# radiocosmology/draco

Hardware: AMD Instinct MI355X
Metric: m-modes/sec through MModeTransform+DirtyMapMaker (128-feed, 256-freq) (higher is better)
Workload: dtype f64 accumulate; B stored complex128; FFT complex64 (as the reference); 1 GPU; cfg3: 128-feed (379 stacked baselines), 256 freq per GPU (256 in the job), 1024 RA, lmax=mmax=512: MModeTransform.process + DirtyMapMaker.process through the task classes (131328 (m,f) solves + alm2map to nside=256 IQUV maps per GPU and day); parallelism=freq-sharded x1, weak scaling (no collective in the timed region)

## Files before the change

draco_amd/csrc/dmm_ctx.hip:

```cpp
#include <stdio.h>
#include <string.h>

#include "dmm_internal.h"

static thread_local char g_err[512] = "";

int dmm_set_error(int code, const char* fmt, ...) {
  va_list ap;
  va_start(ap, fmt);
  vsnprintf(g_err, sizeof(g_err), fmt, ap);
  va_end(ap);
  return code;
}

static const char* const kProfNames[DMM_PROF_NSLOT] = {"gram", "chol", "tridiag", "ql", "backproj", "band", "chase", "solve", "null"};

static void prof_collect(dmm_ctx* c) {
  for (dmm_prof_span& sp : c->prof_open) {
    float ms = 0.f;
    if (hipEventSynchronize(sp.b) == hipSuccess && hipEventElapsedTime(&ms, sp.a, sp.b) == hipSuccess) {
      c->prof_us[sp.slot] += 1e3 * (double)ms;
      ++c->prof_n[sp.slot];
    }
    (void)hipEventDestroy(sp.a);
    (void)hipEventDestroy(sp.b);
  }
  c->prof_open.clear();
}

int dmm_get_scratch(dmm_ctx* ctx, size_t bytes, void** out) {
  if (ctx->scratch_bytes < bytes) {
    if (ctx->scratch) {
      DMM_HIP(hipStreamSynchronize(ctx->stream));
      (void)hipFree(ctx->scratch);
      ctx->scratch = nullptr;
      ctx->scratch_bytes = 0;
    }
    DMM_HIP(hipMalloc(&ctx->scratch, bytes));
    ctx->scratch_bytes = bytes;
  }
  *out = ctx->scratch;
  return DMM_OK;
}

hipError_t dmm_ticket(dmm_ctx* ctx, unsigned long long** out) {
  constexpr int kTickets = 256;
  if (!ctx->ticket) {
    hipError_t e = hipMalloc((void**)&ctx->ticket, kTickets * sizeof(unsigned long long));
    if (e != hipSuccess) return e;
  }
  *out = ctx->ticket + (ctx->ticket_seq++ % kTickets);
  return hipSuccess;
}

extern "C" {

int dmm_version(void) { return DMM_VERSION; }
const char* dmm_last_error(void) { return g_err; }

int dmm_ctx_create(int device, dmm_ctx** out) {
  DMM_REQUIRE(out != nullptr, "dmm_ctx_create: ctx is NULL");
  *out = nullptr;
  int ndev = 0;
  DMM_HIP(hipGetDeviceCount(&ndev));
  DMM_REQUIRE(device >= 0 && device < ndev, "dmm_ctx_create: device %d out of range (%d devices)", device, ndev);
  DMM_HIP(hipSetDevice(device));
  dmm_ctx* c = new (std::nothrow) dmm_ctx();
  if (!c) return dmm_set_error(DMM_E_NOMEM, "dmm_ctx_create: out of host memory");
  c->device = device;
  hipDeviceProp_t prop;
  DMM_HIP(hipGetDeviceProperties(&prop, device));
  c->num_cu = prop.multiProcessorCount > 0 ? prop.multiProcessorCount : 256;
  DMM_HIP(hipEventCreate(&c->ev0));
  DMM_HIP(hipEventCreate(&c->ev1));
  *out = c;
  return DMM_OK;
}

static void free_tables(std::map<int, dmm_fft_tables>& m) {
  for (auto& kv : m) {
    if (kv.second.tw) (void)hipFree(kv.second.tw);
    if (kv.second.chirp) (void)hipFree(kv.second.chirp);
    if (kv.second.bfilt) (void)hipFree(kv.second.bfilt);
  }
  m.clear();
}

int dmm_ctx_destroy(dmm_ctx* c) {
  if (!c) return DMM_OK;
  (void)hipSetDevice(c->device);
  free_tables(c->fft);
  free_tables(c->ifft);
  for (auto& kv : c->sht)
    if (kv.second) (void)hipFree(kv.second);
  prof_collect(c);
  if (c->scratch) (void)hipFree(c->scratch);
  if (c->ticket) (void)hipFree(c->ticket);
  if (c->ev0) (void)hipEventDestroy(c->ev0);
  if (c->ev1) (void)hipEventDestroy(c->ev1);
  for (hipEvent_t e : c->aux_ev)
    if (e) (void)hipEventDestroy(e);
  if (c->aux_stream) (void)hipStreamDestroy(c->aux_stream);
  if (c->aux_stream_b) (void)hipStreamDestroy(c->aux_stream_b);
  if (c->aux_pinned) (void)hipHostFree(c->aux_pinned);
  delete c;
  return DMM_OK;
}

int dmm_ctx_set_stream(dmm_ctx* c, void* s) {
  DMM_REQUIRE(c != nullptr, "dmm_ctx_set_stream: ctx is NULL");
  c->stream = (hipStream_t)s;
  return DMM_OK;
}

int dmm_ctx_set_option(dmm_ctx* c, const char* name, int64_t value) {
  DMM_REQUIRE(c != nullptr && name != nullptr, "dmm_ctx_set_option: NULL argument");
  if (!strcmp(name, "dirty_variant")) c->opt_dirty_variant = (int)value;
  else if (!strcmp(name, "grid_mult")) c->opt_grid_mult = (int)value;
  else if (!strcmp(name, "dirty_static")) c->opt_dirty_static = (int)value;
  else if (!strcmp(name, "dirty_nofill")) c->opt_dirty_nofill = (int)value;
  else if (!strcmp(name, "project_grid_mult")) c->opt_project_grid_mult = (int)value;
  else if (!strcmp(name, "project_variant")) c->opt_project_variant = (int)value;
  else if (!strcmp(name, "ml_inner_sweeps")) c->opt_ml_inner_sweeps = (int)value;
  else if (!strcmp(name, "ml_outer_sweeps")) c->opt_ml_outer_sweeps = (int)value;
  else if (!strcmp(name, "sht_variant")) c->opt_sht_variant = (int)value;
  else if (!strcmp(name, "sht_synth_form")) c->opt_sht_synth_form = (int)value;
  else if (!strcmp(name, "ml_shortcut")) c->opt_ml_shortcut = (int)value;
  else if (!strcmp(name, "ml_null")) c->opt_ml_null = (int)value;
  else if (!strcmp(name, "ml_rank_stop")) c->opt_ml_rank_stop = (int)value;
  else if (!strcmp(name, "ml_chase_split")) c->opt_ml_chase_split = (int)value;
  else if (!strcmp(name, "dirty_prio")) c->opt_dirty_prio = (int)value;
  else if (!strcmp(name, "ml_eigen")) c->opt_ml_eigen = (int)value;
  else if (!strcmp(name, "ringmap_variant")) c->opt_ringmap_variant = (int)value;
  else if (!strcmp(name, "ml_reduce")) c->opt_ml_reduce = (int)value;
  else if (!strcmp(name, "gram_stage")) c->opt_gram_stage = (int)value;
  else if (!strcmp(name, "wiener_overlap")) c->opt_wiener_overlap = (int)value;
  else if (!strcmp(name, "ml_workspace_mib")) c->opt_ml_ws_mib = value > 0 ? value : 0;
  else if (!strcmp(name, "regrid_workspace_mib")) c->opt_regrid_ws_mib = value > 0 ? value : 0;
  else if (!strcmp(name, "wiener_workspace_mib")) c->opt_wiener_ws_mib = value > 0 ? value : 0;
  else if (!strcmp(name, "profile")) {
    prof_collect(c);
    for (int k = 0; k < DMM_PROF_NSLOT; ++k) c->prof_us[k] = 0.0, c->prof_n[k] = 0;
    c->opt_profile = value != 0;
  }
  else return dmm_set_error(DMM_E_ARG, "dmm_ctx_set_option: unknown option '%s'", name);
  return DMM_OK;
}

int dmm_ctx_get_counter(dmm_ctx* c, const char* name, int64_t* value) {
  DMM_REQUIRE(c != nullptr && name != nullptr && value != nullptr, "dmm_ctx_get_counter: NULL argument");
  if (!strcmp(name, "ml_tiles_direct")) *value = c->ml_tiles_direct;
  else if (!strcmp(name, "ml_tiles_eigen")) *value = c->ml_tiles_eigen;
  else if (!strcmp(name, "ml_tiles_null")) *value = c->ml_tiles_null;
  else if (!strcmp(name, "ml_tiles_stopped")) *value = c->ml_tiles_stopped;
  else if (!strcmp(name, "ml_gram_cached")) *value = c->ml_gram_cached;
  else if (!strcmp(name, "ml_tiles_basis")) *value = c->ml_tiles_basis;
  else if (!strcmp(name, "ml_stop_cols")) *value = c->ml_stop_cols;
  else if (!strcmp(name, "ml_gram_flops")) *value = c->ml_gram_flops;
  else if (!strcmp(name, "ml_band_bytes")) *value = c->ml_band_bytes;
  else if (!strcmp(name, "ml_tiles_ql_failed")) *value = c->ml_tiles_ql_failed;
  else if (!strcmp(name, "ml_early_chunks")) *value = c->ml_early_chunks;
  else if (!strcmp(name, "ml_two_stage_max_order")) *value = dmm_ml_two_stage_max_order();
  else if (!strcmp(name, "build_ab")) {
#ifdef DMM_AB
    *value = 1;
#else
    *value = 0;
#endif
  }
  else if (!strcmp(name, "opt_sht_synth_form")) *value = c->opt_sht_synth_form;
  else if (!strncmp(name, "prof_", 5)) {
    const size_t len = strlen(name);
    const bool want_n = len > 7 && !strcmp(name + len - 2, "_n");
    const bool want_us = len > 8 && !strcmp(name + len - 3, "_us");
    int slot = -1;
    for (int k = 0; k < DMM_PROF_NSLOT; ++k) {
      const size_t nl = strlen(kProfNames[k]);
      if (!strncmp(name + 5, kProfNames[k], nl) && name[5 + nl] == '_' && 5 + nl + (want_n ? 2 : 3) == len) slot = k;
    }
    if (slot < 0 || !(want_n || want_us)) return dmm_set_error(DMM_E_ARG, "dmm_ctx_get_counter: unknown counter '%s'", name);
    prof_collect(c);
    *value = want_n ? c->prof_n[slot] : (int64_t)(c->prof_us[slot] + 0.5);
  }
  else return dmm_set_error(DMM_E_ARG, "dmm_ctx_get_counter: unknown counter '%s'", name);
  return DMM_OK;
}

int dmm_ctx_set_ml_basis(dmm_ctx* c, void* U, double* sigma, int32_t* rank, int64_t nslots, int rmax, int build) {
  DMM_REQUIRE(c != nullptr, "dmm_ctx_set_ml_basis: ctx is NULL");
  DMM_REQUIRE(U == nullptr || (sigma != nullptr && rank != nullptr && nslots > 0 && rmax >= 64 && rmax % 64 == 0),
              "dmm_ctx_set_ml_basis: a basis needs sigma, rank, a slot count and rmax a multiple of 64");
  c->ml_bs_U = (double2*)U;
  c->ml_bs_sigma = U ? sigma : nullptr;
  c->ml_bs_rank = U ? rank : nullptr;
  c->ml_bs_slots = U ? nslots : 0;
  c->ml_bs_rmax = U ? rmax : 0;
  c->ml_bs_build = U ? (build == 1) : 0;
  c->ml_bs_rank_h.clear();
  if (U && build == 1) {
    DMM_HIP(hipMemsetAsync(rank, 0xFF, (size_t)nslots * sizeof(int32_t), c->stream));
    c->ml_bs_rank_cache_src = nullptr;
  }
  if (U && build != 1) {
    if (build == 0 && c->ml_bs_rank_cache_src == rank && (int64_t)c->ml_bs_rank_cache.size() == nslots) {
      c->ml_bs_rank_h = c->ml_bs_rank_cache;
    } else {
      c->ml_bs_rank_h.resize((size_t)nslots);
      DMM_HIP(hipMemcpyAsync(c->ml_bs_rank_h.data(), rank, (size_t)nslots * sizeof(int32_t), hipMemcpyDeviceToHost, c->stream));
      DMM_HIP(hipStreamSynchronize(c->stream));
      c->ml_bs_rank_cache = c->ml_bs_rank_h;
      c->ml_bs_rank_cache_src = rank;
    }
  }
  return DMM_OK;
}

int dmm_ctx_set_ml_gram_cache(dmm_ctx* c, void* cache, int32_t* valid, int64_t nslots, int reset) {
  DMM_REQUIRE(c != nullptr, "dmm_ctx_set_ml_gram_cache: ctx is NULL");
  DMM_REQUIRE(cache == nullptr || (valid != nullptr && nslots > 0), "dmm_ctx_set_ml_gram_cache: a cache needs its valid flags and a slot count");
  c->ml_gcache = (double2*)cache;
  c->ml_gvalid = cache ? valid : nullptr;
  c->ml_gslots = cache ? nslots : 0;
  if (cache && reset) DMM_HIP(hipMemsetAsync(valid, 0, (size_t)nslots * sizeof(int32_t), c->stream));
  if (cache && (reset || cache != c->ml_gcache_last || (int64_t)c->ml_gvalid_h.size() != nslots)) c->ml_gvalid_h.assign((size_t)nslots, 0);
  if (cache) c->ml_gcache_last = cache;
  return DMM_OK;
}

int dmm_ctx_set_ml_diag(dmm_ctx* c, double* diag) {
  DMM_REQUIRE(c != nullptr, "dmm_ctx_set_ml_diag: ctx is NULL");
  c->ml_diag = diag;
  return DMM_OK;
}

int dmm_ctx_sync(dmm_ctx* c) {
  DMM_REQUIRE(c != nullptr, "dmm_ctx_sync: ctx is NULL");
  DMM_HIP(hipStreamSynchronize(c->stream));
  if (c->aux_stream) DMM_HIP(hipStreamSynchronize(c->aux_stream));
  if (c->aux_stream_b) DMM_HIP(hipStreamSynchronize(c->aux_stream_b));
  return DMM_OK;
}

int dmm_timer_start(dmm_ctx* c) {
  DMM_REQUIRE(c != nullptr, "dmm_timer_start: ctx is NULL");
  DMM_HIP(hipEventRecord(c->ev0, c->stream));
  return DMM_OK;
}

int dmm_timer_stop(dmm_ctx* c, float* ms) {
  DMM_REQUIRE(c != nullptr && ms != nullptr, "dmm_timer_stop: NULL argument");
  DMM_HIP(hipEventRecord(c->ev1, c->stream));
  DMM_HIP(hipEventSynchronize(c->ev1));
  DMM_HIP(hipEventElapsedTime(ms, c->ev0, c->ev1));
  return DMM_OK;
}

}
```

draco_amd/csrc/dmm_internal.h:

```cpp
#pragma once
#include <hip/hip_runtime.h>
#include <stdint.h>
#include <stdarg.h>
#include <map>
#include <vector>

#include "draco_amd.h"

struct dmm_fft_tables {
  int n = 0;
  int M = 0;
  float2* tw = nullptr;
  float2* chirp = nullptr;
  float2* bfilt = nullptr;
};

enum dmm_prof_slot { DMM_PROF_GRAM = 0, DMM_PROF_CHOL, DMM_PROF_TRIDIAG, DMM_PROF_QL, DMM_PROF_BACKPROJ, DMM_PROF_BAND, DMM_PROF_CHASE, DMM_PROF_SOLVE, DMM_PROF_NULL, DMM_PROF_NSLOT };
struct dmm_prof_span {
  hipEvent_t a, b;
  int slot;
};

struct dmm_ctx {
  int device = 0;
  hipStream_t stream = nullptr;
  hipEvent_t ev0 = nullptr, ev1 = nullptr;
  hipStream_t aux_stream = nullptr;
  hipStream_t aux_stream_b = nullptr;
  hipEvent_t aux_ev[4] = {nullptr, nullptr, nullptr, nullptr};
  int* aux_pinned = nullptr;
  size_t aux_pinned_n = 0;
  int num_cu = 256;
  std::map<int, dmm_fft_tables> fft;
  std::map<int, dmm_fft_tables> ifft;
  std::map<int64_t, void*> sht;
  int opt_dirty_variant = 0;
  int opt_grid_mult = 0;
  int opt_dirty_prio = 0;
  int opt_dirty_static = 0;
  int opt_dirty_nofill = 0;
  int opt_project_grid_mult = 0;
  int opt_project_variant = 0;
  int opt_ml_inner_sweeps = 0, opt_ml_outer_sweeps = 0;
  int opt_sht_variant = 0;
  int opt_sht_synth_form = 0;
  int opt_ml_eigen = 0;
  int64_t opt_regrid_ws_mib = 0;
  int64_t opt_ml_ws_mib = 0, opt_wiener_ws_mib = 0;
  int opt_ml_shortcut = 0;
  int ml_probe_every = 8;
  double ml_pass_rate = 1.0;
  int opt_ml_null = 0;
  int64_t ml_gram_flops = 0, ml_band_bytes = 0;
  int64_t ml_tiles_null = 0;
  int opt_ml_chase_split = 0;
  int opt_ml_rank_stop = 0;
  int64_t ml_order_hist[17] = {};
  int64_t ml_tiles_stopped = 0, ml_stop_cols = 0;
  int64_t ml_tiles_direct = 0, ml_tiles_eigen = 0;
  int64_t ml_tiles_ql_failed = 0;
  int opt_ringmap_variant = 0;
  int opt_wiener_overlap = 1;
  int opt_gram_stage = 0;
  int opt_ml_reduce = 0;
  double2* ml_bs_U = nullptr;
  double* ml_bs_sigma = nullptr;
  int32_t* ml_bs_rank = nullptr;
  int64_t ml_bs_slots = 0;
  int ml_bs_rmax = 0, ml_bs_build = 0;
  std::vector<int32_t> ml_bs_rank_h;
  std::vector<int32_t> ml_bs_rank_cache;
  const int32_t* ml_bs_rank_cache_src = nullptr;
  int64_t ml_tiles_basis = 0;
  double2* ml_gcache = nullptr;
  int32_t* ml_gvalid = nullptr;
  int64_t ml_gslots = 0;
  const void* ml_gcache_last = nullptr;
  std::vector<char> ml_gvalid_h;
  int64_t ml_gram_cached = 0;
  double* ml_diag = nullptr;
  int opt_profile = 0;
  std::vector<dmm_prof_span> prof_open;
  double prof_us[DMM_PROF_NSLOT] = {};
  int64_t prof_n[DMM_PROF_NSLOT] = {};
  int64_t ml_early_chunks = 0;
  unsigned long long* ticket = nullptr;
  unsigned ticket_seq = 0;
  void* scratch = nullptr;
  size_t scratch_bytes = 0;
};

int dmm_get_scratch(dmm_ctx* ctx, size_t bytes, void** out);
hipError_t dmm_ticket(dmm_ctx* ctx, unsigned long long** out);

struct dmm_plan {
  dmm_ctx* ctx = nullptr;
  int64_t ntile = 0;
  int npairs = 0, npol = 0, lmax = 0, nfreq = 0, n_m = 0, b_dtype = 0, b_layout = 0;
  std::vector<dmm_tile> tiles_h;
  dmm_tile* tiles_d = nullptr;
  int32_t* work_start_d = nullptr;
  int32_t* work_rows_d = nullptr;
  int64_t nwork = 0, nwork_rows = 0;
  int cols_per_block = 0;
  int pair_ok = 0;
  int64_t b_bytes = 0;
  std::vector<int16_t> ml_ne;
};

struct dmm_aux_scope {
  dmm_ctx* c;
  explicit dmm_aux_scope(dmm_ctx* ctx) : c(ctx) {}
  dmm_aux_scope(const dmm_aux_scope&) = delete;
  dmm_aux_scope& operator=(const dmm_aux_scope&) = delete;
  ~dmm_aux_scope() {
    if (c && c->aux_stream) (void)hipStreamSynchronize(c->aux_stream);
    if (c && c->aux_stream_b) (void)hipStreamSynchronize(c->aux_stream_b);
  }
};

struct dmm_prof_scope {
  dmm_ctx* c;
  hipStream_t st;
  dmm_prof_span sp;
  bool on;
  dmm_prof_scope(dmm_ctx* ctx, int slot, hipStream_t stream) : c(ctx), st(stream), on(false) {
    if (!c->opt_profile) return;
    sp.slot = slot;
    if (hipEventCreate(&sp.a) != hipSuccess) return;
    if (hipEventCreate(&sp.b) != hipSuccess) {
      (void)hipEventDestroy(sp.a);
      return;
    }
    (void)hipEventRecord(sp.a, st);
    on = true;
  }
  dmm_prof_scope(const dmm_prof_scope&) = delete;
  dmm_prof_scope& operator=(const dmm_prof_scope&) = delete;
  ~dmm_prof_scope() {
    if (!on) return;
    (void)hipEventRecord(sp.b, st);
    c->prof_open.push_back(sp);
  }
};

int dmm_set_error(int code, const char* fmt, ...);
#define DMM_HIP(call)                                                                  \
  do {                                                                                 \
    hipError_t e_ = (call);                                                            \
    if (e_ != hipSuccess)                                                              \
      return dmm_set_error((int)e_, "%s failed: %s (%s:%d)", #call, hipGetErrorString(e_), \
                           __FILE__, __LINE__);                                        \
  } while (0)
#define DMM_REQUIRE(cond, ...)                                \
  do {                                                        \
    if (!(cond)) return dmm_set_error(DMM_E_ARG, __VA_ARGS__); \
  } while (0)

int dmm_fft_tables_f64(dmm_ctx* ctx, int n, dmm_fft_tables** out);
void dmm_dirty_tile_list(const dmm_plan* pl, const int64_t* ids, int n, std::vector<dmm_tile>& tiles, std::vector<int32_t>& work);
int dmm_dirty_launch_list(dmm_plan* pl, const void* B, const void* mvis, const double* mweight, const dmm_tile* tiles_d,
                          const int32_t* work_d, int nmat, int64_t nwork, void* alm);
int dmm_dirty_w_launch_list(dmm_plan* pl, const void* B, const double2* wbuf, const double* Sl, const dmm_tile* tiles_d,
                            const int32_t* work_d, int nmat, int64_t nwork, void* alm);
int dmm_ml_two_stage_max_order();

static inline bool dmm_is_pow2(int n) { return n > 0 && (n & (n - 1)) == 0; }
static inline int ilog2(int n) {
  int l = 0;
  while ((1 << l) < n) ++l;
  return l;
}
```

draco_amd/csrc/sht.hip:

```cpp
#include "sht_common.h"
#include "sht_legendre.h"
#include "sht_rings.h"

namespace {

int get_geom(dmm_ctx* ctx, int nside, int lmax, int mmax, ShtGeom* out) {
  const int64_t key = ((int64_t)nside << 40) | ((int64_t)lmax << 20) | (int64_t)mmax;
  auto it = ctx->sht.find(key);
  const int nring = 4 * nside - 1;
  const size_t nd = (size_t)3 * nring + (mmax + 1);
  const size_t bytes = nd * sizeof(double) + (size_t)nring * sizeof(int64_t) + (size_t)nring * sizeof(int);
  const size_t coef_ofs = (bytes + 63) / 64 * 64;
  const size_t coef_rows = (size_t)coef_row0(mmax + 1, lmax);
  int blue_rmax = 0;
  std::vector<int64_t> bf_off(1, 0);
  int64_t bf_total = 0;
  for (int ir = 1; ir < nside && blue_len(ir) <= kMaxBlue; ++ir) {
    bf_off.push_back(bf_total);
    bf_total += blue_len(ir);
    blue_rmax = ir;
  }
  const size_t bfo_ofs = coef_ofs + coef_rows * sizeof(Coef);
  const size_t bf_ofs = (bfo_ofs + bf_off.size() * sizeof(int64_t) + 63) / 64 * 64;
  const size_t phase_ofs = (bf_ofs + (size_t)bf_total * sizeof(double2) + 63) / 64 * 64;
// ... 90 lines not shown
  g.blue_rmax = blue_rmax;
  g.phase = reinterpret_cast<double2*>(gb + phase_ofs);
  g.tw = reinterpret_cast<double2*>(gb + tw_ofs);
  g.tw_len = tw_len;
  g.chirp = reinterpret_cast<double2*>(gb + chirp_ofs);
  *out = g;
  return DMM_OK;
}

int check_args(const char* who, dmm_ctx* ctx, const void* a, const void* b, int nfreq, int npol, int lmax, int mmax,
               int nside) {
  DMM_REQUIRE(ctx && a && b, "%s: NULL argument", who);
  DMM_REQUIRE(nfreq >= 1 && lmax >= 0 && mmax >= 0 && mmax <= lmax, "%s: bad sizes nfreq=%d lmax=%d mmax=%d", who, nfreq, lmax, mmax);
  DMM_REQUIRE(npol == 1 || npol == 4, "%s: npol must be 1 or 4 (got %d)", who, npol);
  DMM_REQUIRE(nside >= 1 && (nside & (nside - 1)) == 0 && nside <= 8192, "%s: nside must be a power of two (got %d)", who, nside);
  return DMM_OK;
}

size_t chunk_freqs(int nfreq, int npol, int nring, int mmax) {
  const size_t grp = npol == 4 ? kSynF : 1;
  const size_t per_f = (size_t)npol * nring * (mmax + 1) * sizeof(double2);
  size_t nf = ((size_t)1 << 30) / per_f / grp * grp;
  if (nf < grp) nf = grp;
  if (nf > (size_t)nfreq) nf = nfreq;
  const size_t nchunk = ((size_t)nfreq + nf - 1) / nf;
  const size_t c = ((size_t)nfreq + nchunk - 1) / nchunk;
  return c < (size_t)nfreq ? (c + grp - 1) / grp * grp : c;
}

size_t coef_scratch_bytes(size_t nfc, int npol, int nring, int mmax) {
  const size_t nfs = npol == 4 ? (nfc + kSynF - 1) / kSynF * kSynF : nfc;
  return nfs * npol * nring * (size_t)(mmax + 1) * sizeof(double2);
}

struct ClassLaunch {
  RingClass rc;
  int nblock;
  int nphi_max;
  bool blue;
};

std::vector<ClassLaunch> ring_classes(const ShtGeom& g) {
  std::vector<ClassLaunch> out;
  ClassLaunch b;
  b.rc.belt = 1;
  b.rc.r_lo = b.rc.r_hi = 0;
  b.rc.M = 4 * g.nside;
  b.rc.logM = 0;
  while ((1 << b.rc.logM) < b.rc.M) ++b.rc.logM;
  b.nblock = 2 * g.nside + 1;
  b.nphi_max = 4 * g.nside;
  b.blue = false;
  out.push_back(b);
  for (int ir = 1; ir < g.nside;) {
    const int M = blue_len(ir);
    int hi = ir;
    while (hi + 1 < g.nside && blue_len(hi + 1) == M) ++hi;
    ClassLaunch c;
    c.rc.belt = 0;
    c.rc.r_lo = ir;
    c.rc.r_hi = hi;
    c.rc.M = M;
    c.rc.logM = 0;
    while ((1 << c.rc.logM) < M) ++c.rc.logM;
    c.nblock = 2 * (hi - ir + 1);
    c.nphi_max = 4 * hi;
    c.blue = true;
    out.push_back(c);
    ir = hi + 1;
  }
  return out;
}

size_t ring_fft_lds(const ShtGeom& g, const ClassLaunch& c, int nrow, int force_direct) {
  if (force_direct) return 0;
  if (c.blue && c.rc.r_hi > g.blue_rmax) return 0;
  const size_t lds = ((size_t)nrow * (c.rc.M + 1) + c.rc.M / 2 + (c.blue ? c.nphi_max : 0)) * sizeof(double2);
  return lds <= 160 * 1024 ? lds : 0;
}

size_t ring_synth_lds(const ShtGeom& g, const ClassLaunch& c, int nb, bool stage_all, int force_direct) {
  if (force_direct) return 0;
  if (c.blue && c.rc.r_hi > g.blue_rmax) return 0;
  const int nm = g.mmax + 1;
  const bool staged = stage_all || 4 * (c.blue ? c.rc.r_lo : g.nside) < nm;
  const size_t lds = ((size_t)nb * (c.rc.M + 1) + c.rc.M / 2 + (c.blue ? c.nphi_max : 0) + (staged ? (size_t)nb * 2 * nm : 0)) *
                     sizeof(double2);
  return lds <= 160 * 1024 ? lds : 0;
}

using RingKernel = void (*)(RingParams, RingClass);

int launch_ring(RingKernel kern, dim3 grid, int threads, size_t lds, hipStream_t st, const RingParams& rp, const RingClass& rc) {
  if (lds > 160 * 1024) return dmm_set_error(DMM_E_UNSUPPORTED, "SHT ring stage needs %zu bytes of LDS (nside too large)", lds);
  DMM_HIP(hipFuncSetAttribute((const void*)kern, hipFuncAttributeMaxDynamicSharedMemorySize, (int)lds));
  hipLaunchKernelGGL(kern, grid, dim3(threads), lds, st, rp, rc);
  DMM_HIP(hipGetLastError());
  return DMM_OK;
}

RingParams ring_params(const ShtGeom& g, int nf, int npol, double2* b, double* map, const double* map_ref) {
  RingParams rp;
  rp.g = g;
  rp.nf = nf;
  rp.npol = npol;
  rp.b = b;
  rp.map = map;
  rp.map_ref = map_ref;
  rp.npix = 12LL * g.nside * g.nside;
  rp.stage_all = 0;
  return rp;
}

#define DMM_BY_NPOL(npol, f, ...) ((npol) == 4 ? f<4>(__VA_ARGS__) : f<1>(__VA_ARGS__))

template <int NPOL>
int synth_chunk(dmm_ctx* ctx, const ShtGeom& g, const double2* alm, int n_m, int nf, double2* b, double* map) {
  LegParams lp;
  lp.g = g;
  lp.nf = nf;
  lp.npol = NPOL;
  lp.n_m = n_m;
  lp.alm = alm;
  lp.b = b;
  if (NPOL == 4 && !(ctx->opt_sht_variant & 8)) {
    const int npair = (g.nring + 1) / 2;
    const int nrc = (npair + kThreads - 1) / kThreads;
    const int nx = g.mmax + 1;
    const int64_t col_bytes = (int64_t)4 * n_m * (g.lmax + 1) * (int64_t)sizeof(double2);
    const bool fits8 = 2 * kLegF * col_bytes < ((int64_t)1 << 32), fits4 = kLegF * col_bytes < ((int64_t)1 << 32);
    if ((ctx->opt_sht_variant & 64) || ctx->opt_sht_synth_form == 1 || !fits4) {
      const int nz = (nf + kLegF - 1) / kLegF;
      hipLaunchKernelGGL(k_leg_synth_mfma, dim3(nx, nrc, nz), dim3(kThreads), 0, ctx->stream, lp);
    } else if ((ctx->opt_sht_variant & 128) || !fits8) {
      const int nz = (nf + kLegF - 1) / kLegF;
      hipLaunchKernelGGL(k_leg_synth_mfma2<1>, dim3(nx, nrc, nz), dim3(kThreads), 0, ctx->stream, lp);
    } else {
      const int nz = (nf + 2 * kLegF - 1) / (2 * kLegF);
      hipLaunchKernelGGL(k_leg_synth_mfma2<2>, dim3(nx, nrc, nz), dim3(kThreads), 0, ctx->stream, lp);
    }
  } else {
    hipLaunchKernelGGL(k_leg_synth<NPOL>, dim3(g.mmax + 1, nf), dim3(kThreads), 0, ctx->stream, lp);
  }
  DMM_HIP(hipGetLastError());
  RingParams rp = ring_params(g, nf, NPOL, b, map, nullptr);
  constexpr int KF = NPOL == 4 ? kSynF : 1;
  const dim3 per_ring((nf + KF - 1) / KF, NPOL == 4 ? 2 : 1);
  const int force_direct = ctx->opt_sht_variant & 4;
  constexpr int N2 = NPOL == 4 ? 2 : 1, N4 = NPOL == 4 ? 4 : 1;
  static const RingKernel fft_kernel[3][2] = {{k_ring_synth_fft<NPOL, 1, false>, k_ring_synth_fft<NPOL, 1, true>},
                                              {k_ring_synth_fft<NPOL, N2, false>, k_ring_synth_fft<NPOL, N2, true>},
                                              {k_ring_synth_fft<NPOL, N4, false>, k_ring_synth_fft<NPOL, N4, true>}};
  for (const ClassLaunch& c : ring_classes(g)) {
    int nb = 0;
    size_t lds = 0;
    rp.stage_all = 0;
    for (int tier = 0; tier < 3 && nb == 0; ++tier)
      for (int b = KF; b >= 1 && nb == 0; b >>= 1) {
        const size_t l = ring_synth_lds(g, c, b, tier == 0, force_direct);
        if (l != 0 && l <= (tier < 2 ? (size_t)80 * 1024 : (size_t)160 * 1024)) nb = b, lds = l, rp.stage_all = tier == 0;
      }
    const int rc = nb == 0 ? launch_ring(k_ring_synth<NPOL>, dim3(c.nblock, nf), kThreads, (size_t)NPOL * (g.mmax + 1) * sizeof(double2),
                                         ctx->stream, rp, c.rc)
                           : launch_ring(fft_kernel[nb >> 1][c.blue], dim3(c.nblock, per_ring.x, per_ring.y), kFftThreads, lds,
                                         ctx->stream, rp, c.rc);
    if (rc) return rc;
  }
  return DMM_OK;
}

template <int NPOL>
int anal_chunk(dmm_ctx* ctx, const ShtGeom& g, const double* map, int n_m, int nf, double2* b, double2* alm, int accumulate,
               const double* map_ref = nullptr) {
  const RingParams rp = ring_params(g, nf, NPOL, b, const_cast<double*>(map), map_ref);
  constexpr int NROWS = NPOL == 4 ? 2 : 1;
  const int force_direct = ctx->opt_sht_variant & 4;
  static const RingKernel fft_kernel[2][2] = {{k_ring_anal_fft<NPOL, 1, false>, k_ring_anal_fft<NPOL, 1, true>},
                                              {k_ring_anal_fft<NPOL, NROWS, false>, k_ring_anal_fft<NPOL, NROWS, true>}};
  for (const ClassLaunch& c : ring_classes(g)) {
    const size_t lds2 = ring_fft_lds(g, c, NROWS, force_direct), lds1 = ring_fft_lds(g, c, 1, force_direct);
    const bool both = NROWS == 2 && lds2 != 0 && lds2 <= 80 * 1024;
    const int rc = lds1 == 0 ? launch_ring(k_ring_anal<NPOL>, dim3(c.nblock, nf), kThreads, (size_t)NPOL * c.nphi_max * sizeof(double),
                                           ctx->stream, rp, c.rc)
                             : launch_ring(fft_kernel[both][c.blue], dim3(c.nblock, nf, both ? 1 : NROWS), kFftThreads,
                                           both ? lds2 : lds1, ctx->stream, rp, c.rc);
    if (rc) return rc;
  }
  LegAnalParams lp;
  lp.g = g;
  lp.nf = nf;
  lp.npol = NPOL;
  lp.n_m = n_m;
  lp.b = b;
  lp.alm = alm;
  lp.accumulate = accumulate;
  if (NPOL == 4 && !(ctx->opt_sht_variant & 8)) {
    hipLaunchKernelGGL(k_leg_anal_mfma, dim3(g.mmax + 1, (nf + kLegF - 1) / kLegF), dim3(kThreads), 0, ctx->stream, lp);
    DMM_HIP(hipGetLastError());
    return DMM_OK;
  }
  constexpr int NV = NPOL == 4 ? 8 : 2;
  const size_t lds2 = (size_t)(g.lmax + 1) * NV * sizeof(double) + (size_t)2 * (kThreads / 64) * kAnalBatch * NV * sizeof(double);
  DMM_HIP(hipFuncSetAttribute((const void*)k_leg_anal<NPOL>, hipFuncAttributeMaxDynamicSharedMemorySize, (int)lds2));
  hipLaunchKernelGGL(k_leg_anal<NPOL>, dim3(g.mmax + 1, nf), dim3(kThreads), lds2, ctx->stream, lp);
  DMM_HIP(hipGetLastError());
  return DMM_OK;
}

}

extern "C" {

int dmm_alm2map(dmm_ctx* ctx, const void* alm, int nfreq, int npol, int lmax, int mmax, int nside, double* map) {
  int rc = check_args("dmm_alm2map", ctx, alm, map, nfreq, npol, lmax, mmax, nside);
  if (rc) return rc;
  DMM_HIP(hipSetDevice(ctx->device));
  ShtGeom g;
  rc = get_geom(ctx, nside, lmax, mmax, &g);
  if (rc) return rc;
  const size_t nfc = chunk_freqs(nfreq, npol, g.nring, mmax);
  void* scratch = nullptr;
  rc = dmm_get_scratch(ctx, coef_scratch_bytes(nfc, npol, g.nring, mmax), &scratch);
  if (rc) return rc;
  const int64_t npix = 12LL * nside * nside;
  const int n_m = mmax + 1;
  for (int f0 = 0; f0 < nfreq; f0 += (int)nfc) {
    const int nf = (int)((size_t)(nfreq - f0) < nfc ? (size_t)(nfreq - f0) : nfc);
    const double2* a = (const double2*)alm + (int64_t)f0 * npol * n_m * (lmax + 1);
    double* mp = map + (int64_t)f0 * npol * npix;
    rc = DMM_BY_NPOL(npol, synth_chunk, ctx, g, a, n_m, nf, (double2*)scratch, mp);
    if (rc) return rc;
  }
  return DMM_OK;
}

int dmm_map2alm(dmm_ctx* ctx, const double* map, int nfreq, int npol, int lmax, int mmax, int nside, int niter,
                void* alm) {
  int rc = check_args("dmm_map2alm", ctx, map, alm, nfreq, npol, lmax, mmax, nside);
  if (rc) return rc;
  DMM_REQUIRE(niter >= 0 && niter <= 64, "dmm_map2alm: niter=%d out of range", niter);
  if ((size_t)npol * 4 * nside * sizeof(double) > 150 * 1024)
    return dmm_set_error(DMM_E_UNSUPPORTED, "dmm_map2alm: nside=%d too large for the in-LDS ring stage", nside);
  DMM_HIP(hipSetDevice(ctx->device));
  ShtGeom g;
  rc = get_geom(ctx, nside, lmax, mmax, &g);
  if (rc) return rc;
  const int64_t npix = 12LL * nside * nside;
  size_t nfc = chunk_freqs(nfreq, npol, g.nring, mmax);
  const size_t b_bytes = coef_scratch_bytes(nfc, npol, g.nring, mmax);
  const size_t r_bytes = niter > 0 ? nfc * npol * (size_t)npix * sizeof(double) : 0;
  void* scratch = nullptr;
  rc = dmm_get_scratch(ctx, b_bytes + r_bytes, &scratch);
  if (rc) return rc;
  double2* b = (double2*)scratch;
  double* resid = (double*)((unsigned char*)scratch + b_bytes);
  const int n_m = mmax + 1;
  for (int f0 = 0; f0 < nfreq; f0 += (int)nfc) {
    const int nf = (int)((size_t)(nfreq - f0) < nfc ? (size_t)(nfreq - f0) : nfc);
    double2* a = (double2*)alm + (int64_t)f0 * npol * n_m * (lmax + 1);
    const double* mp = map + (int64_t)f0 * npol * npix;
    rc = DMM_BY_NPOL(npol, anal_chunk, ctx, g, mp, n_m, nf, b, a, 0);
    if (rc) return rc;
    for (int it = 0; it < niter; ++it) {
      rc = DMM_BY_NPOL(npol, synth_chunk, ctx, g, a, n_m, nf, b, resid);
      if (rc) return rc;
      rc = DMM_BY_NPOL(npol, anal_chunk, ctx, g, resid, n_m, nf, b, a, 1, mp);
      if (rc) return rc;
    }
  }
  return DMM_OK;
}

}
```

draco_amd/csrc/sht_rings.h:

```cpp
#pragma once
#include "sht_common.h"

namespace {

struct RingParams {
  ShtGeom g;
  int nf, npol;
  double2* b;
  double* map;
  int64_t npix;
  const double* map_ref;
  int stage_all;
};

struct RingClass {
  int belt;
  int r_lo, r_hi;
  int M, logM;
};
constexpr int kMinBlue = 256, kMaxBlue = 4096;

__host__ __device__ __forceinline__ int blue_len(int ir) {
  int M = kMinBlue;
  while (M < 8 * ir - 1) M <<= 1;
  return M;
}

__device__ __forceinline__ int class_ring(const RingClass& rc, const ShtGeom& g, int i) {
  if (rc.belt) return g.nside - 1 + i;
  const int ir = rc.r_lo + (i >> 1);
  return (i & 1) ? g.nring - ir : ir - 1;
}

template <int NPOL>
__global__ __launch_bounds__(kThreads) void k_ring_synth(RingParams p, RingClass rc) {
  extern __shared__ __align__(16) unsigned char smem[];
  double2* c = reinterpret_cast<double2*>(smem);
  const int ring = class_ring(rc, p.g, blockIdx.x);
  const int f = blockIdx.y;
  const int nm = p.g.mmax + 1;
  const double phi0 = p.g.phi0[ring];
  const int nphi = p.g.nphi[ring];
  for (int idx = threadIdx.x; idx < NPOL * nm; idx += kThreads) {
    const int pol = idx / nm, m = idx - pol * nm;
    double2 v;
    if (NPOL == 1) {
      v = p.b[((int64_t)f * p.g.nring + ring) * nm + m];
    } else {
      const double* q = reinterpret_cast<const double*>(p.b) + syn4_at(f, m, ring, pol >> 1, p.g.nring, nm) + syn4_slot(pol);
      v = make_double2(q[0], q[2]);
    }
    double sn, cs;
    sincos((double)m * phi0, &sn, &cs);
    const double fac = m == 0 ? 1.0 : 2.0;
    c[idx] = make_double2(fac * (v.x * cs - v.y * sn), fac * (v.x * sn + v.y * cs));
  }
  __syncthreads();
  const int64_t base = p.g.start[ring];
  for (int j = threadIdx.x; j < nphi; j += kThreads) {
    double sn, cs;
    sincospi(2.0 * (double)j / (double)nphi, &sn, &cs);
    double pr = 1.0, pi_ = 0.0;
    double acc[NPOL];
#pragma unroll
    for (int q = 0; q < NPOL; ++q) acc[q] = 0.0;
    for (int m = 0; m < nm; ++m) {
#pragma unroll
      for (int q = 0; q < NPOL; ++q) {
        const double2 cm = c[q * nm + m];
        acc[q] = fma(cm.x, pr, fma(-cm.y, pi_, acc[q]));
      }
      const double nr = pr * cs - pi_ * sn;
      pi_ = fma(pr, sn, pi_ * cs);
      pr = nr;
    }
#pragma unroll
    for (int q = 0; q < NPOL; ++q) p.map[((int64_t)f * NPOL + q) * p.npix + base + j] = acc[q];
  }
}

constexpr int kFftThreads = 256;

struct RingLds {
  dmm_fft::C<double>* buf;
  dmm_fft::C<double>* tw;
  dmm_fft::C<double>* chirp;
};

template <int NROW, bool BLUE>
__device__ __forceinline__ RingLds ring_lds(unsigned char* smem, const ShtGeom& g, int N, int M) {
  RingLds l;
  l.buf = reinterpret_cast<dmm_fft::C<double>*>(smem);
  l.tw = l.buf + NROW * (M + 1);
  l.chirp = l.tw + (M >> 1);
  const int stride = g.tw_len / M;
  for (int k = threadIdx.x; k < (M >> 1); k += kFftThreads) {
    const double2 t = g.tw[k * stride];
    l.tw[k] = {t.x, t.y};
  }
  if (BLUE) {
    const int ir = N >> 2;
    const double2* src = g.chirp + (int64_t)2 * ir * (ir - 1);
    for (int k = threadIdx.x; k < N; k += kFftThreads) {
      const double2 t = src[k];
      l.chirp[k] = {t.x, t.y};
    }
  }
  return l;
}

__global__ void k_fill_ring_tables(const double* phi0, int nring, int mmax, double2* phase, double2* tw, int tw_len,
                                   double2* chirp) {
  const int b = blockIdx.x;
  if (b < nring) {
    const double p0 = phi0[b];
    for (int m = threadIdx.x; m <= mmax; m += blockDim.x) {
      double sn, cs;
      sincos((double)m * p0, &sn, &cs);
      phase[(int64_t)b * (mmax + 1) + m] = make_double2(cs, sn);
    }
  } else if (b == nring) {
    for (int k = threadIdx.x; k < tw_len / 2; k += blockDim.x) {
      double sn, cs;
      sincospi(-2.0 * (double)k / (double)tw_len, &sn, &cs);
      tw[k] = make_double2(cs, sn);
    }
  } else {
    const int ir = b - nring, N = 4 * ir;
    double2* dst = chirp + (int64_t)2 * ir * (ir - 1);
    for (int k = threadIdx.x; k < N; k += blockDim.x) {
      const int k2 = (int)(((int64_t)k * k) % (2 * (int64_t)N));
      double sn, cs;
      sincospi(-(double)k2 / (double)N, &sn, &cs);
      dst[k] = make_double2(cs, sn);
    }
  }
}

template <int NROW, bool BLUE>
__device__ __forceinline__ void ring_dft(const RingLds& l, const double2* bfilt, int M, int logM) {
  const int P = M + 1;
  if (BLUE) dmm_fft::bluestein_convolve<double, kFftThreads>(l.buf, l.tw, bfilt, NROW, M, logM, P, true);
  else dmm_fft::fft_dif8<double, kFftThreads>(l.buf, l.tw, NROW, M, logM, P);
}

template <bool BLUE>
__device__ __forceinline__ dmm_fft::C<double> ring_dft_at(const RingLds& l, int r, int k, int M, int logM) {
  if (BLUE) return dmm_fft::cmul<double>(l.buf[r * (M + 1) + k], l.chirp[k]);
  return l.buf[r * (M + 1) + dmm_fft::bitrev(k, logM)];
}

template <int NPOL, int NB, bool BLUE>
__global__ __launch_bounds__(kFftThreads) void k_ring_synth_fft(RingParams p, RingClass rc) {
  using dmm_fft::C;
  constexpr int KF = NPOL == 4 ? kSynF : 1;
  static_assert(KF % NB == 0, "passes of NB transforms");
  extern __shared__ __align__(16) unsigned char smem[];
  const int ring = class_ring(rc, p.g, blockIdx.x), r = NPOL == 4 ? (int)blockIdx.z : 0;
  const int f0 = KF * blockIdx.y, nfb = min(KF, p.nf - f0);
  const int n = p.g.nphi[ring], M = rc.M, P = M + 1;
  const RingLds l = ring_lds<NB, BLUE>(smem, p.g, n, M);
  if (BLUE) __syncthreads();
  const int nm = p.g.mmax + 1;
  const double2* phase = p.g.phase + (int64_t)ring * nm;
  auto load = [&](int fi, int m, double2& va, double2& vb) {
    if (NPOL == 1) {
      va = p.b[((int64_t)(f0 + fi) * p.g.nring + ring) * nm + m];
    } else {
      const double* q = reinterpret_cast<const double*>(p.b) + syn4_at(f0 + fi, m, ring, r, p.g.nring, nm);
      const double2 re = *reinterpret_cast<const double2*>(q), im = *reinterpret_cast<const double2*>(q + 2);
      va = r == 0 ? make_double2(re.x, im.x) : make_double2(re.y, im.y);
      vb = r == 0 ? make_double2(re.y, im.y) : make_double2(re.x, im.x);
    }
  };
  const bool staged = p.stage_all || n < nm;
  C<double>* rot = l.chirp + (BLUE ? 4 * rc.r_hi : 0);
  const double2* bfilt = BLUE ? p.g.bfilt + p.g.bf_off[rc.belt ? 0 : rc.r_lo + ((int)blockIdx.x >> 1)] : nullptr;
  const int64_t base = p.g.start[ring];
  for (int fb = 0; fb < nfb; fb += NB) {
    if (fb > 0) __syncthreads();
    if (staged) {
      for (int q = threadIdx.x; q < NB * nm; q += kFftThreads) {
        const int m = q / NB, j = q - m * NB;
        C<double> a = {0.0, 0.0}, b = {0.0, 0.0};
        if (fb + j < nfb) {
          const double2 ph = phase[m];
          const double cs = ph.x, sn = ph.y;
          double2 va, vb;
          load(fb + j, m, va, vb);
          a = {va.x * cs - va.y * sn, va.x * sn + va.y * cs};
          if (NPOL == 4) b = {vb.x * cs - vb.y * sn, vb.x * sn + vb.y * cs};
          if (m == 0) a.y = b.y = 0.0;
        }
        rot[(j * 2 + 0) * nm + m] = a;
        rot[(j * 2 + 1) * nm + m] = b;
      }
      __syncthreads();
    }
    for (int k = threadIdx.x; k < M; k += kFftThreads) {
      double zr[NB], zi[NB];
#pragma unroll
      for (int j = 0; j < NB; ++j) zr[j] = zi[j] = 0.0;
      if (k < n && staged) {
        for (int m = k; m < nm; m += n) {
#pragma unroll
          for (int j = 0; j < NB; ++j) {
            const C<double> a = rot[(j * 2 + 0) * nm + m], b = rot[(j * 2 + 1) * nm + m];
            zr[j] += a.x - b.y;
            zi[j] += a.y + b.x;
          }
        }
        for (int m = (k == 0 ? n : n - k); m < nm; m += n) {
#pragma unroll
          for (int j = 0; j < NB; ++j) {
            const C<double> a = rot[(j * 2 + 0) * nm + m], b = rot[(j * 2 + 1) * nm + m];
            zr[j] += a.x + b.y;
            zi[j] += b.x - a.y;
          }
        }
      } else if (k < n) {
        for (int m = k; m < nm; m += n) {
          const double2 ph = phase[m];
          const double cs = ph.x, sn = ph.y;
#pragma unroll
          for (int j = 0; j < NB; ++j) {
            if (fb + j >= nfb) continue;
            double2 va, vb;
            load(fb + j, m, va, vb);
            double ar = va.x * cs - va.y * sn, ai = va.x * sn + va.y * cs;
            double br = 0.0, bi = 0.0;
            if (NPOL == 4) {
              br = vb.x * cs - vb.y * sn;
              bi = vb.x * sn + vb.y * cs;
            }
            if (m == 0) ai = bi = 0.0;
            zr[j] += ar - bi;
            zi[j] += ai + br;
          }
        }
        for (int m = (k == 0 ? n : n - k); m < nm; m += n) {
          const double2 ph = phase[m];
          const double cs = ph.x, sn = ph.y;
#pragma unroll
          for (int j = 0; j < NB; ++j) {
            if (fb + j >= nfb) continue;
            double2 va, vb;
            load(fb + j, m, va, vb);
            const double ar = va.x * cs - va.y * sn, ai = va.x * sn + va.y * cs;
            double br = 0.0, bi = 0.0;
            if (NPOL == 4) {
              br = vb.x * cs - vb.y * sn;
              bi = vb.x * sn + vb.y * cs;
            }
            zr[j] += ar + bi;
            zi[j] += br - ai;
          }
        }
      }
#pragma unroll
      for (int j = 0; j < NB; ++j) {
        C<double> v = {zr[j], -zi[j]};
        if (BLUE && k < n) v = dmm_fft::cmul<double>(v, l.chirp[k]);
        l.buf[j * P + k] = v;
      }
    }
    __syncthreads();
    ring_dft<NB, BLUE>(l, bfilt, M, rc.logM);
    for (int j = threadIdx.x; j < n; j += kFftThreads) {
#pragma unroll
      for (int jj = 0; jj < NB; ++jj) {
        if (fb + jj >= nfb) continue;
        const int64_t f = f0 + fb + jj;
        const C<double> y = ring_dft_at<BLUE>(l, jj, j, M, rc.logM);
        p.map[(f * NPOL + 2 * r) * p.npix + base + j] = y.x;
        if (NPOL == 4) p.map[(f * NPOL + 2 * r + 1) * p.npix + base + j] = -y.y;
      }
    }
  }
}

template <int NPOL>
__global__ __launch_bounds__(kThreads) void k_ring_anal(RingParams p, RingClass rc) {
  extern __shared__ __align__(16) unsigned char smem[];
  double* px = reinterpret_cast<double*>(smem);
  const int ring = class_ring(rc, p.g, blockIdx.x), f = blockIdx.y;
  const int nm = p.g.mmax + 1;
  const double phi0 = p.g.phi0[ring];
  const int nphi = p.g.nphi[ring];
  const int64_t base = p.g.start[ring];
  for (int idx = threadIdx.x; idx < NPOL * nphi; idx += kThreads) {
    const int pol = idx / nphi, j = idx - pol * nphi;
    const int64_t pi = ((int64_t)f * NPOL + pol) * p.npix + base + j;
    px[idx] = p.map_ref ? p.map_ref[pi] - p.map[pi] : p.map[pi];
  }
  __syncthreads();
  const double w = 4.0 * M_PI / (double)p.npix;
  for (int m = threadIdx.x; m < nm; m += kThreads) {
    double sn, cs;
    sincospi(-2.0 * (double)(m % nphi) / (double)nphi, &sn, &cs);
    double pr = 1.0, pi_ = 0.0;
    double are[NPOL], aim[NPOL];
#pragma unroll
    for (int q = 0; q < NPOL; ++q) are[q] = aim[q] = 0.0;
    for (int j = 0; j < nphi; ++j) {
#pragma unroll
      for (int q = 0; q < NPOL; ++q) {
        const double v = px[q * nphi + j];
        are[q] = fma(v, pr, are[q]);
        aim[q] = fma(v, pi_, aim[q]);
      }
      const double nr = pr * cs - pi_ * sn;
      pi_ = fma(pr, sn, pi_ * cs);
      pr = nr;
    }
    double s0, c0;
    sincos(-(double)m * phi0, &s0, &c0);
#pragma unroll
    for (int q = 0; q < NPOL; ++q)
      p.b[(((int64_t)f * NPOL + q) * p.g.nring + ring) * nm + m] =
          make_double2(w * (are[q] * c0 - aim[q] * s0), w * (are[q] * s0 + aim[q] * c0));
  }
}

template <int NPOL, int NROW, bool BLUE>
__global__ __launch_bounds__(kFftThreads) void k_ring_anal_fft(RingParams p, RingClass rc) {
  using dmm_fft::C;
  extern __shared__ __align__(16) unsigned char smem[];
  const int rb = blockIdx.z * NROW;
  const int ring = class_ring(rc, p.g, blockIdx.x), f = blockIdx.y;
  const int n = p.g.nphi[ring], M = rc.M, P = M + 1;
  const RingLds l = ring_lds<NROW, BLUE>(smem, p.g, n, M);
  if (BLUE) __syncthreads();
  const int64_t base = p.g.start[ring];
  for (int k = threadIdx.x; k < M; k += kFftThreads) {
#pragma unroll
    for (int r = 0; r < NROW; ++r) {
      C<double> v = {0.0, 0.0};
      if (k < n) {
        const int64_t p0 = ((int64_t)f * NPOL + (NPOL == 4 ? 2 * (r + rb) : 0)) * p.npix + base + k, p1 = p0 + p.npix;
        v.x = p.map_ref ? p.map_ref[p0] - p.map[p0] : p.map[p0];
        if (NPOL == 4) v.y = p.map_ref ? p.map_ref[p1] - p.map[p1] : p.map[p1];
        if (BLUE) v = dmm_fft::cmul<double>(v, l.chirp[k]);
      }
      l.buf[r * P + k] = v;
    }
  }
  __syncthreads();
  const double2* bfilt = BLUE ? p.g.bfilt + p.g.bf_off[rc.belt ? 0 : rc.r_lo + ((int)blockIdx.x >> 1)] : nullptr;
  ring_dft<NROW, BLUE>(l, bfilt, M, rc.logM);
  const int nm = p.g.mmax + 1;
  const double2* phase = p.g.phase + (int64_t)ring * nm;
  const double w = 4.0 * M_PI / (double)p.npix;
  for (int m = threadIdx.x; m < nm; m += kFftThreads) {
    const int k = m % n, k2 = (n - k) % n;
    const double2 ph = phase[m];
    const double c0 = ph.x, s0 = -ph.y;
#pragma unroll
    for (int r = 0; r < NROW; ++r) {
      const C<double> X = ring_dft_at<BLUE>(l, r, k, M, rc.logM), Y = ring_dft_at<BLUE>(l, r, k2, M, rc.logM);
      const double ar = 0.5 * (X.x + Y.x), ai = 0.5 * (X.y - Y.y);
      p.b[(((int64_t)f * NPOL + (NPOL == 4 ? 2 * (r + rb) : 0)) * p.g.nring + ring) * nm + m] =
          make_double2(w * (ar * c0 - ai * s0), w * (ar * s0 + ai * c0));
      if (NPOL == 4) {
        const double br = 0.5 * (X.y + Y.y), bi = -0.5 * (X.x - Y.x);
        p.b[(((int64_t)f * NPOL + 2 * (r + rb) + 1) * p.g.nring + ring) * nm + m] =
            make_double2(w * (br * c0 - bi * s0), w * (br * s0 + bi * c0));
      }
    }
  }
}

__global__ __launch_bounds__(kFftThreads) void k_build_bfilt(double2* table, const int64_t* bf_off) {
  using dmm_fft::C;
  extern __shared__ __align__(16) unsigned char smem[];
  const int ir = blockIdx.x + 1, N = 4 * ir, M = blue_len(ir), P = M + 1;
  int logM = 0;
  while ((1 << logM) < M) ++logM;
  C<double>* buf = reinterpret_cast<C<double>*>(smem);
  C<double>* tw = buf + P;
  for (int k = threadIdx.x; k < (M >> 1); k += kFftThreads) {
    double sn, cs;
    sincospi(-2.0 * (double)k / (double)M, &sn, &cs);
    tw[k] = {cs, sn};
  }
  for (int j = threadIdx.x; j < M; j += kFftThreads) {
    const int nn = j < N ? j : (j > M - N ? M - j : -1);
    C<double> v = {0.0, 0.0};
    if (nn >= 0) {
      const int k2 = (int)(((int64_t)nn * nn) % (2 * (int64_t)N));
      double sn, cs;
      sincospi((double)k2 / (double)N, &sn, &cs);
      v = {cs, sn};
    }
    buf[j] = v;
  }
  __syncthreads();
  dmm_fft::fft_dif<double, kFftThreads>(buf, tw, 1, M, logM, P);
  const double inv = 1.0 / (double)M;
  double2* out = table + bf_off[ir];
  for (int k = threadIdx.x; k < M; k += kFftThreads) out[k] = make_double2(buf[k].x * inv, buf[k].y * inv);
}

}
```

Baseline: 2077 m-modes/s.

## Restructure ring-synthesis FFT input fill with direct/mirrored scatter and held registers

For the 4-polarisation unstaged ring-synthesis path, the per-k gather loop that reloaded the harmonic coefficients for each aliased m is replaced with a two-pass scatter. A direct pass writes each rotated coefficient into the FFT buffer, and a mirrored pass adds the conjugate contribution. The first few per-thread values are kept in registers so the mirrored pass does not refetch them from global memory. NPOL=4 now skips the fully staged LDS tier and gains a tunable LDS budget, the NPOL=1 path is specialised to a single frequency, and launch counters are added; the cost is more register pressure and an extra barrier per batch.

```diff
diff --git a/draco_amd/csrc/dmm_ctx.hip b/draco_amd/csrc/dmm_ctx.hip
--- a/draco_amd/csrc/dmm_ctx.hip
+++ b/draco_amd/csrc/dmm_ctx.hip
@@ -125,6 +125,7 @@
   else if (!strcmp(name, "ml_outer_sweeps")) c->opt_ml_outer_sweeps = (int)value;
   else if (!strcmp(name, "sht_variant")) c->opt_sht_variant = (int)value;
   else if (!strcmp(name, "sht_synth_form")) c->opt_sht_synth_form = (int)value;
+  else if (!strcmp(name, "sht_ring_lds_bytes")) c->opt_sht_ring_lds = value > 0 ? value : 0;
   else if (!strcmp(name, "ml_shortcut")) c->opt_ml_shortcut = (int)value;
   else if (!strcmp(name, "ml_null")) c->opt_ml_null = (int)value;
   else if (!strcmp(name, "ml_rank_stop")) c->opt_ml_rank_stop = (int)value;
@@ -169,6 +170,13 @@
 #endif
   }
   else if (!strcmp(name, "opt_sht_synth_form")) *value = c->opt_sht_synth_form;
+  else if (!strncmp(name, "sht_ring_staged_nb", 18) || !strncmp(name, "sht_ring_unstaged_nb", 20)) {
+    const bool st = name[9] == 's';
+    const char* d = name + (st ? 18 : 20);
+    const int lg = !strcmp(d, "1") ? 0 : !strcmp(d, "2") ? 1 : !strcmp(d, "4") ? 2 : -1;
+    if (lg < 0) return dmm_set_error(DMM_E_ARG, "dmm_ctx_get_counter: unknown counter '%s'", name);
+    *value = c->sht_ring_launches[st][lg];
+  }
   else if (!strncmp(name, "prof_", 5)) {
     const size_t len = strlen(name);
     const bool want_n = len > 7 && !strcmp(name + len - 2, "_n");
diff --git a/draco_amd/csrc/dmm_internal.h b/draco_amd/csrc/dmm_internal.h
--- a/draco_amd/csrc/dmm_internal.h
+++ b/draco_amd/csrc/dmm_internal.h
@@ -44,6 +44,8 @@
   int opt_ml_inner_sweeps = 0, opt_ml_outer_sweeps = 0;
   int opt_sht_variant = 0;
   int opt_sht_synth_form = 0;
+  int64_t opt_sht_ring_lds = 0;
+  int64_t sht_ring_launches[2][3] = {};
   int opt_ml_eigen = 0;
   int64_t opt_regrid_ws_mib = 0;
   int64_t opt_ml_ws_mib = 0, opt_wiener_ws_mib = 0;
diff --git a/draco_amd/csrc/sht.hip b/draco_amd/csrc/sht.hip
--- a/draco_amd/csrc/sht.hip
+++ b/draco_amd/csrc/sht.hip
@@ -266,14 +266,16 @@
                                               {k_ring_synth_fft<NPOL, N2, false>, k_ring_synth_fft<NPOL, N2, true>},
                                               {k_ring_synth_fft<NPOL, N4, false>, k_ring_synth_fft<NPOL, N4, true>}};
   for (const ClassLaunch& c : ring_classes(g)) {
+    const size_t budget = ctx->opt_sht_ring_lds > 0 ? (size_t)ctx->opt_sht_ring_lds : (size_t)80 * 1024;
     int nb = 0;
     size_t lds = 0;
     rp.stage_all = 0;
-    for (int tier = 0; tier < 3 && nb == 0; ++tier)
+    for (int tier = NPOL == 4 ? 1 : 0; tier < 3 && nb == 0; ++tier)
       for (int b = KF; b >= 1 && nb == 0; b >>= 1) {
         const size_t l = ring_synth_lds(g, c, b, tier == 0, force_direct);
-        if (l != 0 && l <= (tier < 2 ? (size_t)80 * 1024 : (size_t)160 * 1024)) nb = b, lds = l, rp.stage_all = tier == 0;
+        if (l != 0 && l <= (tier < 2 ? budget : (size_t)160 * 1024)) nb = b, lds = l, rp.stage_all = tier == 0;
       }
+    if (nb) ++ctx->sht_ring_launches[rp.stage_all || 4 * (c.blue ? c.rc.r_lo : g.nside) <= g.mmax][nb >> 1];
     const int rc = nb == 0 ? launch_ring(k_ring_synth<NPOL>, dim3(c.nblock, nf), kThreads, (size_t)NPOL * (g.mmax + 1) * sizeof(double2),
                                          ctx->stream, rp, c.rc)
                            : launch_ring(fft_kernel[nb >> 1][c.blue], dim3(c.nblock, per_ring.x, per_ring.y), kFftThreads, lds,
diff --git a/draco_amd/csrc/sht_rings.h b/draco_amd/csrc/sht_rings.h
--- a/draco_amd/csrc/sht_rings.h
+++ b/draco_amd/csrc/sht_rings.h
@@ -150,6 +150,17 @@
   return l.buf[r * (M + 1) + dmm_fft::bitrev(k, logM)];
 }
 
+
+__device__ __forceinline__ void ring_rotate(const double2& va, const double2& vb, const double2& ph, int m, dmm_fft::C<double>& a,
+                                            dmm_fft::C<double>& b) {
+  const double cs = ph.x, sn = ph.y;
+  a = {va.x * cs - va.y * sn, va.x * sn + va.y * cs};
+  b = {vb.x * cs - vb.y * sn, vb.x * sn + vb.y * cs};
+  if (m == 0) a.y = b.y = 0.0;
+}
+
+constexpr int kHeld = 9;
+
 template <int NPOL, int NB, bool BLUE>
 __global__ __launch_bounds__(kFftThreads) void k_ring_synth_fft(RingParams p, RingClass rc) {
   using dmm_fft::C;
@@ -163,105 +174,145 @@
   if (BLUE) __syncthreads();
   const int nm = p.g.mmax + 1;
   const double2* phase = p.g.phase + (int64_t)ring * nm;
-  auto load = [&](int fi, int m, double2& va, double2& vb) {
-    if (NPOL == 1) {
-      va = p.b[((int64_t)(f0 + fi) * p.g.nring + ring) * nm + m];
-    } else {
-      const double* q = reinterpret_cast<const double*>(p.b) + syn4_at(f0 + fi, m, ring, r, p.g.nring, nm);
-      const double2 re = *reinterpret_cast<const double2*>(q), im = *reinterpret_cast<const double2*>(q + 2);
-      va = r == 0 ? make_double2(re.x, im.x) : make_double2(re.y, im.y);
-      vb = r == 0 ? make_double2(re.y, im.y) : make_double2(re.x, im.x);
-    }
-  };
   const bool staged = p.stage_all || n < nm;
   C<double>* rot = l.chirp + (BLUE ? 4 * rc.r_hi : 0);
   const double2* bfilt = BLUE ? p.g.bfilt + p.g.bf_off[rc.belt ? 0 : rc.r_lo + ((int)blockIdx.x >> 1)] : nullptr;
   const int64_t base = p.g.start[ring];
+  auto fetch = [&](int f, int m, C<double>& a, C<double>& b) {
+    const double* q = reinterpret_cast<const double*>(p.b) + syn4_at(f0 + f, m, ring, r, p.g.nring, nm);
+    const double2 re = *reinterpret_cast<const double2*>(q), im = *reinterpret_cast<const double2*>(q + 2);
+    const double2 va = r == 0 ? make_double2(re.x, im.x) : make_double2(re.y, im.y);
+    const double2 vb = r == 0 ? make_double2(re.y, im.y) : make_double2(re.x, im.x);
+    ring_rotate(va, vb, phase[m], m, a, b);
+  };
   for (int fb = 0; fb < nfb; fb += NB) {
     if (fb > 0) __syncthreads();
-    if (staged) {
-      for (int q = threadIdx.x; q < NB * nm; q += kFftThreads) {
-        const int m = q / NB, j = q - m * NB;
-        C<double> a = {0.0, 0.0}, b = {0.0, 0.0};
-        if (fb + j < nfb) {
-          const double2 ph = phase[m];
-          const double cs = ph.x, sn = ph.y;
-          double2 va, vb;
-          load(fb + j, m, va, vb);
-          a = {va.x * cs - va.y * sn, va.x * sn + va.y * cs};
-          if (NPOL == 4) b = {vb.x * cs - vb.y * sn, vb.x * sn + vb.y * cs};
-          if (m == 0) a.y = b.y = 0.0;
+    auto each_slot = [&](auto&& body) {
+      for (int q = threadIdx.x; q < NB * nm; q += kFftThreads) body(q / NB, q % NB, fb + q % NB < nfb);
+    };
+    if (NPOL == 4 && !staged) {
+      for (int k = nm + threadIdx.x; k < M; k += kFftThreads) {
+#pragma unroll
+        for (int j = 0; j < NB; ++j) l.buf[j * P + k] = {0.0, 0.0};
+      }
+      constexpr int H = NB == KF ? kHeld : 0;
+      C<double> ha[H + 1], hb[H + 1];
+      auto direct = [&](int m, int j, bool live, C<double>& a, C<double>& b) {
+#pragma clang fp contract(off)
+        C<double> z = {0.0, 0.0};
+        if (live) {
+          fetch(fb + j, m, a, b);
+          z.x += a.x - b.y;
+          z.y += a.y + b.x;
         }
-        rot[(j * 2 + 0) * nm + m] = a;
-        rot[(j * 2 + 1) * nm + m] = b;
+        l.buf[j * P + m] = z;
+      };
+      auto mirrored = [&](int m, int j, const C<double>& a, const C<double>& b) {
+#pragma clang fp contract(off)
+        C<double> z = l.buf[j * P + n - m];
+        z.x += a.x + b.y;
+        z.y += b.x - a.y;
+        l.buf[j * P + n - m] = z;
+      };
+#pragma unroll
+      for (int i = 0; i < H; ++i) {
+        const int q = threadIdx.x + kFftThreads * i;
+        if (q < NB * nm) direct(q / NB, q % NB, fb + q % NB < nfb, ha[i], hb[i]);
+      }
+      for (int q = threadIdx.x + kFftThreads * H; q < NB * nm; q += kFftThreads) {
+        C<double> a, b;
+        direct(q / NB, q % NB, fb + q % NB < nfb, a, b);
       }
       __syncthreads();
-    }
-    for (int k = threadIdx.x; k < M; k += kFftThreads) {
-      double zr[NB], zi[NB];
-#pragma unroll
-      for (int j = 0; j < NB; ++j) zr[j] = zi[j] = 0.0;
-      if (k < n && staged) {
-        for (int m = k; m < nm; m += n) {
-#pragma unroll
-          for (int j = 0; j < NB; ++j) {
-            const C<double> a = rot[(j * 2 + 0) * nm + m], b = rot[(j * 2 + 1) * nm + m];
-            zr[j] += a.x - b.y;
-            zi[j] += a.y + b.x;
+#pragma unroll
+      for (int i = 0; i < H; ++i) {
+        const int q = threadIdx.x + kFftThreads * i;
+        if (q < NB * nm && q / NB != 0 && fb + q % NB < nfb) mirrored(q / NB, q % NB, ha[i], hb[i]);
+      }
+      for (int q = threadIdx.x + kFftThreads * H; q < NB * nm; q += kFftThreads) {
+        if (q / NB == 0 || fb + q % NB >= nfb) continue;
+        C<double> a, b;
+        fetch(fb + q % NB, q / NB, a, b);
+        mirrored(q / NB, q % NB, a, b);
+      }
+      __syncthreads();
+      for (int k = threadIdx.x; k < M; k += kFftThreads) {
+#pragma unroll
+        for (int j = 0; j < NB; ++j) {
+          const C<double> z = l.buf[j * P + k];
+          C<double> v = {z.x, -z.y};
+          if (BLUE && k < n) v = dmm_fft::cmul<double>(v, l.chirp[k]);
+          l.buf[j * P + k] = v;
+        }
+      }
+    } else {
+      if (staged) {
+        if (NPOL == 4) {
+          each_slot([&](int m, int j, bool live) {
+            C<double> a = {0.0, 0.0}, b = {0.0, 0.0};
+            if (live) fetch(fb + j, m, a, b);
+            rot[(j * 2 + 0) * nm + m] = a;
+            rot[(j * 2 + 1) * nm + m] = b;
+          });
+        } else {
+          for (int m = threadIdx.x; m < nm; m += kFftThreads) {
+            const double2 ph = phase[m];
+            const double cs = ph.x, sn = ph.y;
+            const double2 va = p.b[((int64_t)f0 * p.g.nring + ring) * nm + m];
+            C<double> a = {va.x * cs - va.y * sn, va.x * sn + va.y * cs};
+            if (m == 0) a.y = 0.0;
+            rot[m] = a;
+            rot[nm + m] = {0.0, 0.0};
           }
         }
-        for (int m = (k == 0 ? n : n - k); m < nm; m += n) {
-#pragma unroll
-          for (int j = 0; j < NB; ++j) {
-            const C<double> a = rot[(j * 2 + 0) * nm + m], b = rot[(j * 2 + 1) * nm + m];
-            zr[j] += a.x + b.y;
-            zi[j] += b.x - a.y;
+        __syncthreads();
+      }
+      for (int k = threadIdx.x; k < M; k += kFftThreads) {
+        double zr[NB], zi[NB];
+#pragma unroll
+        for (int j = 0; j < NB; ++j) zr[j] = zi[j] = 0.0;
+        if (k < n && staged) {
+          for (int m = k; m < nm; m += n) {
+#pragma unroll
+            for (int j = 0; j < NB; ++j) {
+              const C<double> a = rot[(j * 2 + 0) * nm + m], b = rot[(j * 2 + 1) * nm + m];
+              zr[j] += a.x - b.y;
+              zi[j] += a.y + b.x;
+            }
+          }
+          for (int m = (k == 0 ? n : n - k); m < nm; m += n) {
+#pragma unroll
+            for (int j = 0; j < NB; ++j) {
+              const C<double> a = rot[(j * 2 + 0) * nm + m], b = rot[(j * 2 + 1) * nm + m];
+              zr[j] += a.x + b.y;
+              zi[j] += b.x - a.y;
+            }
+          }
+        } else if (NPOL == 1 && k < n) {
+          for (int m = k; m < nm; m += n) {
+            const double2 ph = phase[m];
+            const double cs = ph.x, sn = ph.y;
+            const double2 va = p.b[((int64_t)f0 * p.g.nring + ring) * nm + m];
+            double ar = va.x * cs - va.y * sn, ai = va.x * sn + va.y * cs;
+            if (m == 0) ai = 0.0;
+            zr[0] += ar;
+            zi[0] += ai;
+          }
+          for (int m = (k == 0 ? n : n - k); m < nm; m += n) {
+            const double2 ph = phase[m];
+            const double cs = ph.x, sn = ph.y;
+            const double2 va = p.b[((int64_t)f0 * p.g.nring + ring) * nm + m];
+            const double ar = va.x * cs - va.y * sn, ai = va.x * sn + va.y * cs;
+            zr[0] += ar;
+            zi[0] += 0.0 - ai;
           }
         }
-      } else if (k < n) {
-        for (int m = k; m < nm; m += n) {
-          const double2 ph = phase[m];
-          const double cs = ph.x, sn = ph.y;
-#pragma unroll
-          for (int j = 0; j < NB; ++j) {
-            if (fb + j >= nfb) continue;
-            double2 va, vb;
-            load(fb + j, m, va, vb);
-            double ar = va.x * cs - va.y * sn, ai = va.x * sn + va.y * cs;
-            double br = 0.0, bi = 0.0;
-            if (NPOL == 4) {
-              br = vb.x * cs - vb.y * sn;
-              bi = vb.x * sn + vb.y * cs;
-            }
-            if (m == 0) ai = bi = 0.0;
-            zr[j] += ar - bi;
-            zi[j] += ai + br;
-          }
+#pragma unroll
+        for (int j = 0; j < NB; ++j) {
+          C<double> v = {zr[j], -zi[j]};
+          if (BLUE && k < n) v = dmm_fft::cmul<double>(v, l.chirp[k]);
+          l.buf[j * P + k] = v;
         }
-        for (int m = (k == 0 ? n : n - k); m < nm; m += n) {
-          const double2 ph = phase[m];
-          const double cs = ph.x, sn = ph.y;
-#pragma unroll
-          for (int j = 0; j < NB; ++j) {
-            if (fb + j >= nfb) continue;
-            double2 va, vb;
-            load(fb + j, m, va, vb);
-            const double ar = va.x * cs - va.y * sn, ai = va.x * sn + va.y * cs;
-            double br = 0.0, bi = 0.0;
-            if (NPOL == 4) {
-              br = vb.x * cs - vb.y * sn;
-              bi = vb.x * sn + vb.y * cs;
-            }
-            zr[j] += ar + bi;
-            zi[j] += br - ai;
-          }
-        }
-      }
-#pragma unroll
-      for (int j = 0; j < NB; ++j) {
-        C<double> v = {zr[j], -zi[j]};
-        if (BLUE && k < n) v = dmm_fft::cmul<double>(v, l.chirp[k]);
-        l.buf[j * P + k] = v;
       }
     }
     __syncthreads();
```

After: 2070 m-modes/s. No clear change (-0.3%).
